# undistro/trivy

Measured on AMD Instinct MI355X. Metric: GB/s secret-scanned (whole node) at 1/2/4/8 MI355X; findings bit-exact vs CPU, higher is better.
Workload: dtype u8

## Files before the change

trivy_amd/csrc/engine.hip:

```cpp
#include <chrono>
#include <condition_variable>
#include <mutex>
#include <hip/hip_runtime.h>

#include <algorithm>
#include <cstdlib>
#include <cstdio>
#include <cstring>
#include <string>
#include <pthread.h>

#include <thread>
#include <type_traits>

#include "engine.h"
#include "census.h"
#include "fetch.h"
#include "fetch_host.h"
#include "fetch_windows.h"
#include "xform.h"
#include "filter.h"
#include "k1_orform.h"

namespace tsg {

namespace {

constexpr int kScanThreads = 1024;
constexpr int kScanWaves = kScanThreads / 64;

#define HIP_OK(x)                                                   \
  do {                                                              \
    hipError_t e_ = (x);                                            \
    if (e_ != hipSuccess) {                                         \
      err_ = std::string(#x) + ": " + hipGetErrorString(e_);        \
      return false;                                                 \
    }                                                               \
  } while (0)


constexpr uint32_t kK0Run = 16;
struct ClearParams {
  uint32_t* flags;
  uint32_t* kw;
  uint64_t n_kw;
  uint32_t* counters;
  uint32_t* fs_ctr;
  uint32_t* skip_info;
};
__device__ __forceinline__ void clear_words(uint32_t* p, uint64_t n, uint64_t tid, uint64_t nthr) {
  const uint64_t n4 = n / 4;
  for (uint64_t i = tid; i < n4; i += nthr) reinterpret_cast<uint4*>(p)[i] = make_uint4(0, 0, 0, 0);
  if (tid < n % 4) p[4 * n4 + tid] = 0;
}
__global__ __launch_bounds__(256) void chunk_map_kernel(const uint64_t* __restrict__ off, uint32_t n_files,
                                                        uint64_t n_chunks, uint32_t* __restrict__ chunk_file,
                                                        ClearParams Z) {
  {
    const uint64_t tid = uint64_t(blockIdx.x) * blockDim.x + threadIdx.x, nthr = uint64_t(gridDim.x) * blockDim.x;
    clear_words(Z.flags, n_files, tid, nthr);
    clear_words(Z.kw, Z.n_kw, tid, nthr);
    if (tid < kScanCtrWords) {
      Z.counters[tid] = 0;
      if (Z.fs_ctr) Z.fs_ctr[tid] = 0;
      if (Z.skip_info) Z.skip_info[tid] = 0;
    }
  }
  const uint64_t n_runs = (n_chunks + kK0Run - 1) / kK0Run;
  for (uint64_t r = uint64_t(blockIdx.x) * blockDim.x + threadIdx.x; r < n_runs;
       r += uint64_t(gridDim.x) * blockDim.x) {
    const uint64_t c0 = r * kK0Run;
    uint64_t x = c0 * kChunk;
    uint32_t lo = 0, hi = n_files;
    while (hi - lo > 1) {
      const uint32_t mid = (lo + hi) >> 1;
      if (off[mid] <= x) lo = mid;
      else hi = mid;
    }
    uint32_t v[kK0Run];
    uint64_t fe = off[lo + 1];
#pragma unroll
    for (uint32_t i = 0; i < kK0Run; i++) {
      x = (c0 + i) * kChunk;
      while (x >= fe && lo + 1 < n_files) fe = off[++lo + 1];
      v[i] = lo;
    }
    if (c0 + kK0Run <= n_chunks) {
      uint4* d = reinterpret_cast<uint4*>(chunk_file + c0);
#pragma unroll
      for (uint32_t q = 0; q < kK0Run / 4; q++) d[q] = make_uint4(v[4 * q], v[4 * q + 1], v[4 * q + 2], v[4 * q + 3]);
    } else {
      for (uint32_t i = 0; c0 + i < n_chunks; i++) chunk_file[c0 + i] = v[i];
    }
  }
}

__device__ __forceinline__ uint4 load16(const uint8_t* p) { return *reinterpret_cast<const uint4*>(p); }

__device__ __forceinline__ void wave_sync() {
  __builtin_amdgcn_fence(__ATOMIC_RELEASE, "wavefront");
  __builtin_amdgcn_wave_barrier();
  __builtin_amdgcn_fence(__ATOMIC_ACQUIRE, "wavefront");
}

constexpr int kFLane = 64;
constexpr int kFBlocks = kFLane / 16;
constexpr int kFTile = 64 * kFLane;
constexpr int kFFlushAt = 128;
constexpr int kFQueue = kFFlushAt + 64;
constexpr int kFChunks = kFTile / 1024;
#ifndef TSG_K1_NLTILES
#define TSG_K1_NLTILES 16
#endif
constexpr int kFNlTiles = TSG_K1_NLTILES;
#ifndef TSG_K1_WGS
#define TSG_K1_WGS 2
#endif
constexpr int kFWgPerCu = TSG_K1_WGS;
constexpr uint32_t kFGroup = 8;
#ifndef TSG_K1_OR_READAHEAD
#define TSG_K1_OR_READAHEAD 4
#endif
constexpr uint32_t kFReadAheadOr = TSG_K1_OR_READAHEAD;
constexpr int kFWindow = 6;
constexpr int kFWords = 4;
static_assert(kChunk % kFLane == 0 && kChunk / kFLane <= 64, "a newline chunk must be whole lane chunks");
static_assert(kFChunks * kChunk == kFTile && kFChunks == 4, "a tile's newline counts are one u64");


constexpr uint32_t kRunWords = 8;
__host__ __device__ inline uint64_t KeepWords(uint64_t n_tiles) {
  return ((n_tiles + 63) / 64 + kRunWords - 1) / kRunWords * kRunWords;
}

__global__ __launch_bounds__(256) void tile_keep_kernel(const uint64_t* __restrict__ off, uint32_t n_files,
                                                        const uint32_t* __restrict__ chunk_file,
                                                        const uint8_t* __restrict__ skip, uint64_t n_bytes,
                                                        uint64_t n_tiles, uint64_t* __restrict__ keep_bits,
                                                        uint32_t* __restrict__ info) {
  const uint32_t lane = threadIdx.x & 63u;
  const uint64_t stride = uint64_t(gridDim.x) * blockDim.x;
  const uint64_t n_padded = KeepWords(n_tiles) * 64;
  for (uint64_t base = uint64_t(blockIdx.x) * blockDim.x + (threadIdx.x & ~63u); base < n_padded; base += stride) {
    const uint64_t t = base + lane;
    bool keep = false;
    if (t < n_tiles) {
      const uint64_t ts = t * kFTile, te = ts + kFTile < n_bytes ? ts + kFTile : n_bytes;
      uint32_t f = chunk_file[t * kFChunks];
      for (;;) {
        const uint64_t fb = off[f], fe = off[f + 1];
        if (fe > fb && !skip[f]) {
          keep = true;
          break;
        }
        if (fe >= te || f + 1 >= n_files) break;
        f++;
      }
    }
    const uint64_t m = __ballot(keep);
    if (lane == 0) keep_bits[base / 64] = m;
  }
  constexpr uint32_t kStatBlocks = 64;
  if (blockIdx.x >= kStatBlocks) return;
  const uint64_t fstride = uint64_t(gridDim.x < kStatBlocks ? gridDim.x : kStatBlocks) * blockDim.x;
  uint32_t nf = 0;
  uint64_t nb = 0;
  for (uint64_t f = uint64_t(blockIdx.x) * blockDim.x + threadIdx.x; f < n_files; f += fstride)
    if (skip[f]) {
      nf++;
      nb += off[f + 1] - off[f];
    }
#pragma unroll
  for (int x = 1; x < 64; x <<= 1) {
    nf += __shfl_xor(nf, x);
    nb += __shfl_xor(nb, x);
  }
  if (lane == 0 && nf) {
    atomicAdd(&info[kSkFiles], nf);
    atomicAdd(reinterpret_cast<unsigned long long*>(&info[kSkBytes]), static_cast<unsigned long long>(nb));
  }
}

constexpr int kRunThreads = 1024;
__global__ __launch_bounds__(kRunThreads) void tile_runs_kernel(const uint64_t* __restrict__ keep_bits,
                                                                uint64_t n_tiles, uint2* __restrict__ runs,
                                                                uint32_t* __restrict__ info) {
  __shared__ uint32_t s_k[kRunThreads / 64], s_r[kRunThreads / 64];
  const uint32_t tid = threadIdx.x, lane = tid & 63u, wv = tid >> 6;
  const uint64_t n_words = KeepWords(n_tiles);
  const uint64_t per = ((n_words / kRunWords + kRunThreads - 1) / kRunThreads) * kRunWords;
  const uint64_t w0 = per * tid < n_words ? per * tid : n_words;
  const uint64_t w1 = w0 + per < n_words ? w0 + per : n_words;
  const uint64_t carry0 = w0 > 0 && w0 < n_words ? keep_bits[w0 - 1] >> 63 : 0;
  auto load_group = [&](uint64_t w, uint64_t* b) {
    const uint4* g = reinterpret_cast<const uint4*>(keep_bits + w);
#pragma unroll
    for (uint32_t q = 0; q < kRunWords / 2; q++) {
      const uint4 v = g[q];
      b[2 * q] = uint64_t(v.x) | (uint64_t(v.y) << 32);
      b[2 * q + 1] = uint64_t(v.z) | (uint64_t(v.w) << 32);
    }
  };
  uint32_t kept = 0, starts = 0;
  uint64_t carry = carry0;
  for (uint64_t w = w0; w < w1; w += kRunWords) {
    uint64_t g[kRunWords];
    load_group(w, g);
#pragma unroll
    for (uint32_t q = 0; q < kRunWords; q++) {
      const uint64_t b = g[q];
      kept += uint32_t(__popcll(b));
      starts += uint32_t(__popcll(b & ~((b << 1) | carry)));
      carry = b >> 63;
    }
  }
  uint32_t ik = kept, ir = starts;
#pragma unroll
  for (int x = 1; x < 64; x <<= 1) {
    const uint32_t a = __shfl_up(ik, x), b = __shfl_up(ir, x);
    if (lane >= uint32_t(x)) {
      ik += a;
      ir += b;
    }
  }
  if (lane == 63) {
    s_k[wv] = ik;
    s_r[wv] = ir;
  }
  __syncthreads();
  uint32_t bk = 0, br = 0;
  for (uint32_t q = 0; q < wv; q++) {
    bk += s_k[q];
    br += s_r[q];
  }
  uint32_t k = bk + ik - kept, r = br + ir - starts;
  carry = carry0;
  for (uint64_t w = w0; w < w1; w += kRunWords) {
    uint64_t g[kRunWords];
    load_group(w, g);
#pragma unroll
    for (uint32_t q = 0; q < kRunWords; q++) {
      const uint64_t b = g[q];
      for (uint64_t s = b & ~((b << 1) | carry); s; s &= s - 1) {
        const uint32_t bit = uint32_t(__builtin_ctzll(s));
        runs[r++] = make_uint2(uint32_t((w + q) * 64 + bit), k + uint32_t(__popcll(b & ((uint64_t(1) << bit) - 1))));
      }
      k += uint32_t(__popcll(b));
      carry = b >> 63;
    }
  }
  if (tid == kRunThreads - 1) {
    runs[r] = make_uint2(uint32_t(n_tiles), k);
    info[kSkRuns] = r;
    info[kSkKept] = k;
    info[kSkTailKept] = n_tiles ? uint32_t((keep_bits[(n_tiles - 1) / 64] >> ((n_tiles - 1) & 63)) & 1) : 0u;
    info[kSkTiles] = uint32_t(n_tiles);
  }
}

struct FilterParams {
  const uint8_t* arena;
  uint64_t n_bytes;
  const uint2* runs;
  uint32_t* run_info;
  const uint32_t* reach;
  uint32_t diag_mode;
  uint16_t* nl;
  uint32_t* recs;
  uint32_t rec_cap;
  uint32_t* counters;
};

__device__ __forceinline__ uint4 reach_read(const uint8_t* sb, uint32_t w, uint32_t k, uint32_t laneoff) {
  return *reinterpret_cast<const uint4*>(sb + __builtin_amdgcn_perm(w, laneoff, 0x0C0C0000u | ((4u + k) << 8)));
}

__device__ __forceinline__ uint4 reach_read_whole(const uint8_t* sb, uint32_t w, uint32_t k, uint32_t laneoff) {
  uint4 r = reach_read(sb, w, k, laneoff);
  asm volatile("" : "+v"(r.x), "+v"(r.y), "+v"(r.z), "+v"(r.w));
  return r;
}

__device__ __forceinline__ void reach_apply(const uint4& m, uint32_t* st) {
  asm("v_lshl_or_b32 %0, %1, 4, %2" : "=v"(st[0]) : "v"(st[0]), "v"(m.x));
  asm("v_lshl_or_b32 %0, %1, 4, %2" : "=v"(st[1]) : "v"(st[1]), "v"(m.y));
  asm("v_lshl_or_b32 %0, %1, 4, %2" : "=v"(st[2]) : "v"(st[2]), "v"(m.z));
  asm("v_lshl_or_b32 %0, %1, 4, %2" : "=v"(st[3]) : "v"(st[3]), "v"(m.w));
}

__device__ __forceinline__ uint32_t nl_count4(uint32_t w) {
  const uint32_t a = ((w ^ 0x0A0A0A0Au) & 0x7F7F7F7Fu) + 0x7F7F7F7Fu;
  return __popc(~(a | w) & 0x80808080u);
}

__device__ __forceinline__ uint32_t word_of(uint4 v, uint32_t i) {
  return i < 2 ? (i == 0 ? v.x : v.y) : (i == 2 ? v.z : v.w);
}

__device__ __forceinline__ void load_reach_lds(uint8_t* s_reach, const uint32_t* reach, int tid, int nthreads) {
  for (uint32_t i = tid; i < 256; i += nthreads)
    reinterpret_cast<uint4*>(s_reach)[i] = reinterpret_cast<const uint4*>(reach)[i];
}

__device__ __forceinline__ void load_orform_lds(uint8_t* s_reach, const uint32_t* reach, int tid, int nthreads) {
  for (uint32_t i = tid; i < 256 * 4; i += nthreads) {
    const uint32_t b = i >> 2;
    const uint4 r = reinterpret_cast<const uint4*>(reach)[b];
    const uint32_t in[4] = {r.x, r.y, r.z, r.w};
    uint32_t w[4];
    OrFormRow(in, w);
#pragma unroll
    for (uint32_t c = 0; c < 4; c++)
      reinterpret_cast<uint4*>(s_reach)[b * 16 + (i & 3) * 4 + c] = make_uint4(w[0], w[1], w[2], w[3]);
  }
}

__device__ __forceinline__ uint32_t or3_keep(uint32_t a, uint32_t b, uint32_t c) {
  uint32_t h;
  asm("v_or3_b32 %0, %1, %2, %3" : "=v"(h) : "v"(a), "v"(b), "v"(c));
  return h;
}
__device__ __forceinline__ uint32_t and_or_keep(uint32_t acc, uint32_t a, uint32_t b) {
  asm("v_bitop3_b32 %0, %1, %2, %3 bitop3:0xe0" : "=v"(acc) : "v"(acc), "v"(a), "v"(b));
  return acc;
}

template <bool kRuns>
__global__ __launch_bounds__(kScanThreads, 8) void filter_kernel(FilterParams P) {
  __shared__ __attribute__((aligned(16))) uint8_t s_reach[65536];
  __shared__ uint32_t s_queue[kScanWaves * kFQueue];
  __shared__ uint64_t s_nl[kScanWaves * kFNlTiles];
  const int tid = threadIdx.x;
  load_orform_lds(s_reach, P.reach, tid, blockDim.x);
  __syncthreads();
  const uint32_t lane = tid & 63;
  const uint32_t wave = __builtin_amdgcn_readfirstlane(uint32_t(tid) >> 6);
  uint32_t* Q = s_queue + wave * kFQueue;
  uint64_t* NL = s_nl + wave * kFNlTiles;
  auto ln = [&]() {
    uint32_t l = lane;
    asm volatile("" : "+v"(l));
    return l;
  };
  uint32_t nl_slots = 0;
  uint32_t qn = 0;
  const uint64_t n_tiles = (P.n_bytes + kFTile - 1) / kFTile;
  const uint64_t n_waves = uint64_t(gridDim.x) * kScanWaves;
  const uint64_t wid = uint64_t(blockIdx.x) * kScanWaves + wave;
  const uint2* __restrict__ RUNS = kRuns ? P.runs : nullptr;
  auto uni = [](uint32_t v) { return uint32_t(__builtin_amdgcn_readfirstlane(v)); };
  const uint64_t n_kept = RUNS ? uint64_t(uni(P.run_info[kSkKept])) : n_tiles;
  const bool tail_kept = RUNS ? uni(P.run_info[kSkTailKept]) != 0 : true;
  const uint64_t per = n_kept / n_waves, extra = n_kept % n_waves;
  auto uni64 = [&](uint64_t v) { return uint64_t(uni(uint32_t(v))) | uint64_t(uni(uint32_t(v >> 32))) << 32; };
  const uint64_t k_begin = uni64(wid * per + (wid < extra ? wid : extra));
  const uint64_t k_end = uni64(k_begin + per + (wid < extra ? 1 : 0));
  uint32_t run = 0;
  uint64_t run_k1 = n_kept;
  uint64_t t_begin = k_begin;
  uint32_t runs_walked = 1;
  if (RUNS && k_begin < k_end) {
    uint32_t lo = 0, hi = uni(P.run_info[kSkRuns]);
    while (hi - lo > 1) {
      const uint32_t mid = (lo + hi) >> 1;
      if (uni(RUNS[mid].y) <= k_begin) lo = mid;
      else hi = mid;
    }
    run = lo;
    const uint2 r0 = RUNS[lo];
    t_begin = uint64_t(uni(r0.x)) + (k_begin - uni(r0.y));
    run_k1 = uni(RUNS[lo + 1].y);
  }
  uint4 buf[kFBlocks];
  uint32_t pre_x = 0, pre_y = 0;
  auto load_pre = [&](uint64_t tt) {
    const uint2 pv = *reinterpret_cast<const uint2*>(P.arena + tt * kFTile - 8);
    pre_x = __builtin_amdgcn_readfirstlane(pv.x);
    pre_y = __builtin_amdgcn_readfirstlane(pv.y);
  };
  if (k_begin < k_end && t_begin > 0) load_pre(t_begin);
  auto next_tile = [&](uint64_t k1, uint64_t tcur, bool* nr) -> uint64_t {
    if (k1 < run_k1) {
      *nr = false;
      return tcur + 1;
    }
    run++;
    runs_walked++;
    run_k1 = uni(RUNS[run + 1].y);
    *nr = true;
    return uni(RUNS[run].x);
  };
  auto lane_ptr = [&](uint64_t tt) -> const uint8_t* {
    const uint64_t b0 = tt * kFTile + uint64_t(ln()) * kFLane;
    return P.arena + (b0 < P.n_bytes ? b0 : 0);
  };
  auto load_tile = [&](uint4* dst, uint64_t tt) {
    const uint8_t* lp = lane_ptr(tt);
#pragma unroll
    for (int j = 0; j < kFBlocks; j++) dst[j] = load16(lp + 16 * j);
  };
  auto flush = [&]() {
    uint32_t base = 0;
    const uint32_t l = ln();
    if (l == 0) base = atomicAdd(&P.counters[kCtRecs], qn);
    base = __builtin_amdgcn_readfirstlane(base);
    for (uint32_t i = l; i < qn; i += 64) {
      if (base + i < P.rec_cap) P.recs[base + i] = Q[i];
      else P.counters[kCtRecOvf] = 1;
    }
    qn = 0;
  };
  uint32_t fl_acc = 0;
  uint32_t grp_n = 0;
  uint64_t grp_t0 = 0;
  auto compact = [&]() {
    const uint32_t cnt = __popc(fl_acc);
    uint32_t incl = cnt;
    incl += uint32_t(__builtin_amdgcn_update_dpp(0, int(incl), 0x111, 0xF, 0xF, true));
    incl += uint32_t(__builtin_amdgcn_update_dpp(0, int(incl), 0x112, 0xF, 0xF, true));
    incl += uint32_t(__builtin_amdgcn_update_dpp(0, int(incl), 0x114, 0xF, 0xF, true));
    incl += uint32_t(__builtin_amdgcn_update_dpp(0, int(incl), 0x118, 0xF, 0xF, true));
    incl += uint32_t(__builtin_amdgcn_update_dpp(0, int(incl), 0x142, 0xA, 0xF, false));
    incl += uint32_t(__builtin_amdgcn_update_dpp(0, int(incl), 0x143, 0xC, 0xF, false));
    const uint32_t total = __builtin_amdgcn_readlane(incl, 63);
    if (total) {
      if (qn + total > kFQueue) flush();
      const uint32_t l = ln();
      const uint32_t rec0 = __builtin_amdgcn_readfirstlane(uint32_t(grp_t0 * (kFTile / 16))) + l * kFBlocks;
      uint32_t m = fl_acc;
      if (total <= kFQueue) {
        uint32_t at = qn + incl - cnt;
        while (m) {
          const uint32_t b = uint32_t(__builtin_ctz(m));
          m &= m - 1;
          Q[at++] = rec0 + ((b >> 2) << 8) + (b & 3u);
        }
        qn += total;
      } else {
        uint32_t base = 0;
        if (l == 0) base = atomicAdd(&P.counters[kCtRecs], total);
        uint32_t at = __builtin_amdgcn_readfirstlane(base) + incl - cnt;
        while (m) {
          const uint32_t b = uint32_t(__builtin_ctz(m));
          m &= m - 1;
          if (at < P.rec_cap) P.recs[at] = rec0 + ((b >> 2) << 8) + (b & 3u);
          else P.counters[kCtRecOvf] = 1;
          at++;
        }
      }
    }
    fl_acc = 0;
    grp_n = 0;
  };
  auto flush_nl = [&](uint64_t t_last) {
    wave_sync();
    uint32_t l = lane;
    asm volatile("" : "+v"(l));
    if (l < nl_slots) {
      const uint64_t tt = t_last - uint64_t(nl_slots - 1 - l);
      reinterpret_cast<uint64_t*>(P.nl)[tt] = NL[l];
    }
    nl_slots = 0;
  };
  auto tile = [&](uint4* cur, uint64_t tt, auto tail_tag, const uint8_t* nxt = nullptr) {
    constexpr bool kTail = decltype(tail_tag)::value;
    constexpr bool kRefill = !kTail;
    if (kTail) {
      const uint64_t b0 = tt * kFTile + uint64_t(lane) * kFLane;
#pragma unroll
      for (int j = 0; j < kFBlocks; j++) {
        const uint64_t p = b0 + 16 * j;
        uint32_t wd[4] = {cur[j].x, cur[j].y, cur[j].z, cur[j].w};
#pragma unroll
        for (int q = 0; q < 4; q++) {
          const uint64_t wp = p + 4 * q;
          if (wp >= P.n_bytes) wd[q] = 0;
          else if (wp + 4 > P.n_bytes) wd[q] &= (1u << (8 * (P.n_bytes - wp))) - 1u;
        }
        cur[j] = make_uint4(wd[0], wd[1], wd[2], wd[3]);
      }
    }
    const uint32_t p0 = uint32_t(__builtin_amdgcn_update_dpp(int(pre_x), int(cur[kFBlocks - 1].z), 0x138, 0xF, 0xF,
                                                             false));
    const uint32_t p1 = uint32_t(__builtin_amdgcn_update_dpp(int(pre_y), int(cur[kFBlocks - 1].w), 0x138, 0xF, 0xF,
                                                             false));
    pre_x = __builtin_amdgcn_readlane(cur[kFBlocks - 1].z, 63);
    pre_y = __builtin_amdgcn_readlane(cur[kFBlocks - 1].w, 63);
    uint32_t flagged = 0, nl = 0;
    if (P.diag_mode < 2) {
      const uint32_t laneoff = (ln() & 15) * 16;
      constexpr uint32_t kRA = kFReadAheadOr;
      static_assert(kRA % 2 == 0 && 16 % kRA == 0, "positions are combined in pairs");
      uint32_t xh[4], yh[2], hprev;
      {
        auto row = [&](uint32_t w, uint32_t k) { return reach_read_whole(s_reach, w, k, laneoff); };
        const uint4 r5 = row(p0, 3), r4 = row(p1, 0), r3 = row(p1, 1), r2 = row(p1, 2), r1 = row(p1, 3);
        hprev = or3_keep(r5.x, r3.y, r1.z);
        xh[0] = r4.x, xh[1] = r3.x, xh[2] = r2.x, xh[3] = r1.x;
        yh[0] = r2.y, yh[1] = r1.y;
      }
#pragma unroll
      for (int j = 0; j < kFBlocks; j++) {
        const uint32_t wd[4] = {cur[j].x, cur[j].y, cur[j].z, cur[j].w};
        uint32_t acc = ~0u;
#pragma unroll
        for (uint32_t g = 0; g < 16; g += kRA) {
          uint4 m[kRA];
#pragma unroll
          for (uint32_t q = 0; q < kRA; q++) m[q] = reach_read(s_reach, wd[(g + q) >> 2], (g + q) & 3, laneoff);
#pragma unroll
          for (uint32_t q = 0; q < kRA; q += 2) {
            const uint32_t k = g + q;
            const uint32_t h0 = or3_keep(xh[k & 3], yh[0], m[q].z);
            const uint32_t h1 = or3_keep(xh[(k + 1) & 3], yh[1], m[q + 1].z);
            xh[k & 3] = m[q].x, xh[(k + 1) & 3] = m[q + 1].x;
            yh[0] = m[q].y, yh[1] = m[q + 1].y;
            const uint32_t hi = __builtin_amdgcn_perm(h1, h0, 0x07060302u);
            const uint32_t lo = __builtin_amdgcn_perm(h0, hprev, 0x05040100u);
            acc = and_or_keep(acc, hi, lo);
            nl += m[q].w + m[q + 1].w;
            hprev = h1;
          }
        }
        flagged |= uint32_t(acc != ~0u) << j;
        if constexpr (kRefill) cur[j] = load16(nxt + 16 * j);
      }
    } else {
#pragma unroll
      for (int j = 0; j < kFBlocks; j++) {
        nl += nl_count4(cur[j].x) + nl_count4(cur[j].y) + nl_count4(cur[j].z) + nl_count4(cur[j].w);
        if constexpr (kRefill) cur[j] = load16(nxt + 16 * j);
      }
    }
    {
    nl += uint32_t(__builtin_amdgcn_update_dpp(0, int(nl), 0x111, 0xF, 0xF, true));
    nl += uint32_t(__builtin_amdgcn_update_dpp(0, int(nl), 0x112, 0xF, 0xF, true));
    nl += uint32_t(__builtin_amdgcn_update_dpp(0, int(nl), 0x114, 0xF, 0xF, true));
    nl += uint32_t(__builtin_amdgcn_update_dpp(0, int(nl), 0x118, 0xF, 0xF, true));
    static_assert(kChunk / kFLane == 16, "one newline chunk per DPP row");
    static_assert(kFTile / 16 == 256, "a tile's records: 256 blocks");
    const uint32_t l = ln();
    if ((l & 15) == 15) reinterpret_cast<uint16_t*>(NL + nl_slots)[l >> 4] = uint16_t(nl);
    if (++nl_slots == kFNlTiles) flush_nl(tt);
    }
    if (grp_n == 0) grp_t0 = tt;
    fl_acc |= flagged << (4 * grp_n);
    grp_n++;
  };
  auto flush_due = [&]() {
    if (grp_n == kFGroup) compact();
    if (qn >= kFFlushAt) flush();
  };
  using Full = std::false_type;
  if constexpr (!kRuns) {
    const uint64_t t_end = k_end;
    const uint64_t t_full = t_end < P.n_bytes / kFTile ? t_end : P.n_bytes / kFTile;
    uint64_t t = t_begin;
    if (t < t_full) load_tile(buf, t);
    while (t < t_full) {
      flush_due();
      tile(buf, t, Full(), lane_ptr(t + 1 < t_full ? t + 1 : t));
      t++;
    }
    if (t < t_end) {
      flush_due();
      load_tile(buf, t);
      tile(buf, t, std::true_type());
      t++;
    }
    if (grp_n) compact();
    if (qn) flush();
    if (nl_slots) flush_nl(t - 1);
    return;
  }
  const bool partial = (P.n_bytes % kFTile) != 0 && tail_kept;
  const uint64_t k_full = uni64((partial && k_end == n_kept && k_end > k_begin) ? k_end - 1 : k_end);
  uint64_t k = k_begin, t = t_begin, t_prev = t_begin;
  bool nr_cur = false;
  auto run_boundary = [&]() {
    if (grp_n) compact();
    if (nl_slots) flush_nl(t_prev);
  };
  auto step = [&](uint4* cur) {
    if (nr_cur) run_boundary();
    flush_due();
    uint64_t tn = t;
    bool nr_n = false;
    if (k + 1 < k_end) tn = next_tile(k + 1, t, &nr_n);
    if (nr_cur) load_pre(t);
    tile(cur, t, Full(), lane_ptr(k + 1 < k_full ? tn : t));
    t_prev = t;
    t = tn;
    nr_cur = nr_n;
    k++;
  };
  if (k < k_full) load_tile(buf, t);
  while (k < k_full) step(buf);
  if (k < k_end) {
    if (nr_cur) run_boundary();
    flush_due();
    if (nr_cur) load_pre(t);
    load_tile(buf, t);
    tile(buf, t, std::true_type());
    t_prev = t;
    k++;
  }
  if (grp_n) compact();
  if (qn) flush();
  if (nl_slots) flush_nl(t_prev);
  if (RUNS && lane == 0 && k_begin < k_end) atomicMax(&P.run_info[kSkWaveRuns], runs_walked);
}

struct NfaParams {
  const uint8_t* arena;
  const uint64_t* off;
  uint32_t n_files;
  const uint16_t* nl;
  const AnchorInfo* anchors;
  const RuleGpu* rules;
  const uint32_t* rule_kw;
  const uint32_t* kwbits;
  uint32_t kw_words;
  const uint32_t* flags;
  const uint64_t* nfa;
  const uint32_t* hits;
  uint32_t hit_cap;
  uint32_t* counters;
  Candidate* cands;
  uint32_t cand_cap;
  const uint32_t* fullscan_rules;
  uint32_t n_fullscan_rules;
  uint32_t fs_chunk;
  uint32_t kw_fold;
  uint32_t diag;
  const uint8_t* skip;
  uint32_t drop_marked;
};

__device__ __forceinline__ bool kw_bits_inexact(const NfaParams& P, uint32_t f) {
  return (P.flags[f] & 4u) && !(P.kw_fold && P.counters[kCtFoldOvf] == 0);
}



#ifndef TSG_C_THREADS
#define TSG_C_THREADS 512
#endif
constexpr int kCThreads = TSG_C_THREADS;
#ifndef TSG_C_THREADS_G
#define TSG_C_THREADS_G 256
#endif
constexpr int kCThreadsG = TSG_C_THREADS_G;
template <bool kLdsTabs>
constexpr int ConfirmThreads() { return kLdsTabs ? kCThreads : kCThreadsG; }

struct FoldSite {
  uint64_t x;
  uint32_t f;
  uint32_t len;
};

__device__ __forceinline__ uint32_t wave_slot(uint32_t* ctr) {
  const uint64_t m = __ballot(1);
  const uint32_t leader = uint32_t(__ffsll(static_cast<unsigned long long>(m)) - 1);
  const uint32_t rank = __builtin_amdgcn_mbcnt_hi(uint32_t(m >> 32), __builtin_amdgcn_mbcnt_lo(uint32_t(m), 0u));
  uint32_t base = 0;
  if (rank == 0) base = atomicAdd(ctr, uint32_t(__popcll(m)));
  base = __shfl(base, int(leader));
  return base + rank;
}

#ifndef TSG_C_HITS
#define TSG_C_HITS 96
#endif
constexpr uint32_t kCWaveHits = TSG_C_HITS;

constexpr uint32_t kHitAidBits = 24;
__device__ __forceinline__ uint32_t hit_aid_word(uint32_t aid, uint64_t end) {
  return aid | (uint32_t(end >> 32) << kHitAidBits);
}
__host__ __device__ __forceinline__ void hit_unpack(const uint32_t* h, uint32_t* f, uint64_t* end, uint32_t* aid) {
  *f = h[0];
  *end = uint64_t(h[1]) | (uint64_t(h[2] >> kHitAidBits) << 32);
  *aid = h[2] & ((1u << kHitAidBits) - 1u);
}

__device__ __forceinline__ void stage_hit(uint32_t* hbuf, uint32_t* hcnt, uint32_t* hits, uint32_t cap,
                                          uint32_t* counters, uint32_t f, uint64_t end, uint32_t aid) {
  const uint32_t k = atomicAdd(hcnt, 1u);
  if (k < kCWaveHits) {
    hbuf[3 * k + 0] = f;
    hbuf[3 * k + 1] = uint32_t(end);
    hbuf[3 * k + 2] = hit_aid_word(aid, end);
    return;
  }
  const uint32_t g = atomicAdd(&counters[kCtHits], 1u);
  if (g < cap) {
    hits[3ull * g + 0] = f;
    hits[3ull * g + 1] = uint32_t(end);
    hits[3ull * g + 2] = hit_aid_word(aid, end);
  } else {
    counters[kCtHitOvf] = 1;
  }
}

__device__ __forceinline__ void flush_staged(uint32_t* hbuf, uint32_t* hcnt, uint32_t* hits, uint32_t cap,
                                             uint32_t* counters, uint32_t lane) {
  wave_sync();
  const uint32_t n_all = __builtin_amdgcn_readfirstlane(*hcnt);
  const uint32_t n = n_all < kCWaveHits ? n_all : kCWaveHits;
  if (n) {
    uint32_t base = 0;
    if (lane == 0) base = atomicAdd(&counters[kCtHits], n);
    base = __builtin_amdgcn_readfirstlane(base);
    for (uint32_t i = lane; i < n; i += 64) {
      if (base + i < cap) {
        hits[3ull * (base + i) + 0] = hbuf[3 * i + 0];
        hits[3ull * (base + i) + 1] = hbuf[3 * i + 1];
        hits[3ull * (base + i) + 2] = hbuf[3 * i + 2];
      } else {
        counters[kCtHitOvf] = 1;
      }
    }
  }
  wave_sync();
  if (lane == 0) *hcnt = 0;
  wave_sync();
}

__device__ __forceinline__ void put_hit(uint32_t* hits, uint32_t cap, uint32_t* counters, uint32_t f, uint64_t end,
                                        uint32_t aid) {
  const uint32_t g = wave_slot(&counters[kCtHits]);
  if (g < cap) {
    hits[3ull * g + 0] = f;
    hits[3ull * g + 1] = uint32_t(end);
    hits[3ull * g + 2] = hit_aid_word(aid, end);
  } else {
    counters[kCtHitOvf] = 1;
  }
}
__device__ __forceinline__ bool follow_lut_pass(const FollowLut& L, const uint32_t* X, int64_t avail) {
  const uint32_t n0 = L.n[0], n1 = L.n[1];
  if (n0 == 0) return true;
  const int64_t span0 = int64_t(L.hi[0]) + n0, span1 = n1 ? int64_t(L.hi[1]) + n1 : 0;
  const int64_t lim = avail < (span0 > span1 ? span0 : span1) ? avail : (span0 > span1 ? span0 : span1);
  uint32_t nonascii = 0;
#pragma unroll
  for (int j = 0; j < 13; j++) {
    const int64_t v = lim - 4 * j;
    const uint32_t vm = v >= 4 ? ~0u : (v <= 0 ? 0u : (1u << (8 * uint32_t(v))) - 1u);
    nonascii |= X[j] & vm;
  }
  if (nonascii & 0x80808080u) return true;
  uint32_t t[4], h[2];
// ... 2682 lines not shown
    fo.n_items = e.n_fitems_;
    fo.stage_items = e.fold_stage_ ? 1u : 0u;
    fo.n_classes = e.n_fclasses_;
    static const uint32_t fold_diag =
        std::getenv("TSG_DIAG_FOLD") ? uint32_t(std::atoi(std::getenv("TSG_DIAG_FOLD"))) : 0u;
    fo.diag = fold_diag;
    fo.pairs = static_cast<const FoldPair*>(e.d_fold_pairs_);
    fo.first = static_cast<const uint32_t*>(e.d_fold_first_);
    fo.n_pairs_k = e.n_fold_pairs_k_;
    fo.n_pairs_s = e.n_fold_pairs_s_;
    fo.n_cap_k = e.n_fold_cap_k_;
    fo.n_cap_s = e.n_fold_cap_s_;
    fo.folds = static_cast<const FoldSite*>(e.d_folds_);
    fo.fold_cap = e.caps_.fold;
    fo.idx_off = static_cast<const uint32_t*>(e.d_fold_idx_off_);
    fo.idx_items = static_cast<const uint32_t*>(e.d_fold_idx_items_);
    fo.n_cap_k_idx = e.n_fold_cap_k_idx_;
    fo.n_cap_s_idx = e.n_fold_cap_s_idx_;
    fo.hits = static_cast<uint32_t*>(e.d_hits_);
    fo.hit_cap = e.caps_.hit;
    fo.counters = W.counters;
    return fo;
  }
  static KwFoldParams KwFold(const GpuEngine& e, const WorkSet& W, const uint8_t* d_arena,
                             const uint64_t* d_offsets) {
    KwFoldParams kf;
    kf.arena = d_arena;
    kf.off = d_offsets;
    kf.tabs = static_cast<const uint8_t*>(e.d_ftabs_);
    kf.t_items = e.ft_items_;
    kf.t_item_ids = e.ft_item_ids_;
    kf.t_item_cls = e.ft_item_cls_;
    kf.t_classes = e.ft_classes_;
    kf.pairs = static_cast<const FoldPair*>(e.d_kwfold_pairs_);
    kf.n_rng_i = e.n_kwf_ri_;
    kf.n_rng_k = e.n_kwf_rk_;
    kf.n_cap_i = e.n_kwf_ci_;
    kf.n_cap_k = e.n_kwf_ck_;
    kf.folds = static_cast<const FoldSite*>(e.d_folds_);
    kf.fold_cap = e.caps_.fold;
    kf.counters = W.counters;
    kf.kwbits = static_cast<uint32_t*>(W.kw);
    kf.kw_words = e.kw_words_;
    return kf;
  }
  static NfaParams Nfa(const GpuEngine& e, const WorkSet& W, const uint8_t* d_arena, const uint64_t* d_offsets,
                       uint32_t n_files, const SkipIn* skip) {
    NfaParams np;
    np.arena = d_arena;
    np.off = d_offsets;
    np.n_files = n_files;
    np.nl = static_cast<const uint16_t*>(e.d_nl_);
    np.anchors = e.d_anchors_;
    np.rules = e.d_rules_;
    np.rule_kw = e.d_rule_kw_;
    np.kwbits = static_cast<const uint32_t*>(W.kw);
    np.kw_words = e.kw_words_;
    np.flags = static_cast<const uint32_t*>(W.flags);
    np.nfa = e.d_nfa_;
    np.hits = static_cast<const uint32_t*>(e.d_hits_);
    np.hit_cap = e.caps_.hit;
    np.counters = W.counters;
    static const uint32_t verify_diag =
        std::getenv("TSG_DIAG_VERIFY") ? uint32_t(std::atoi(std::getenv("TSG_DIAG_VERIFY"))) : 0u;
    np.diag = verify_diag;
    np.cands = static_cast<Candidate*>(W.cands);
    np.cand_cap = e.caps_.cand;
    np.fullscan_rules = e.d_fullscan_rules_;
    np.n_fullscan_rules = e.n_fullscan_rules_;
    np.fs_chunk = e.fs_chunk_;
    np.skip = skip ? skip->d_skip : nullptr;
    np.drop_marked = skip && skip->drop_marked ? 1u : 0u;
    np.kw_fold = e.kw_fold_ ? 1u : 0u;
    return np;
  }
  static FsLists FullScanLists(const GpuEngine& e, const WorkSet& W) {
    FsLists fq;
    fq.pairs = static_cast<FsPair*>(e.d_fs_pairs_);
    fq.pair_cap = e.caps_.fs_pair;
    fq.tasks = static_cast<FsTask*>(e.d_fs_tasks_);
    fq.task_cap = e.caps_.fs_task;
    fq.wave_pairs = static_cast<uint32_t*>(e.d_fs_wave_);
    fq.ctr = W.fs_ctr;
    fq.task_min = e.caps_.fs_task_bytes;
    return fq;
  }
};

bool GpuEngine::EnqueuePhase(const uint8_t* d_arena, uint64_t n_bytes, const uint64_t* d_offsets, uint32_t n_files,
                             uint64_t n_chunks, WorkSet& W, bool k0_aux, PhaseEvents& E, const SkipIn* skip) {
  const uint64_t f_tiles = (n_bytes + kFTile - 1) / kFTile;
  if (skip && (!skip->d_skip || f_tiles == 0)) skip = nullptr;
  if (!EnsureSets(n_chunks, n_files, f_tiles, skip != nullptr)) return false;
  if (!Ensure(&d_nl_, &cap_nl_, (n_chunks + 8) * 2) ||
      !Ensure(&d_folds_, &cap_folds_, size_t(caps_.fold) * sizeof(FoldSite)) ||
      !Ensure(&d_recs_, &cap_recs_, size_t(caps_.rec) * 4) ||
      !Ensure(&d_hits_, &cap_hits_, size_t(caps_.hit) * 12))
    return false;
  if (n_fullscan_rules_ > 0 &&
      (!Ensure(&d_fs_pairs_, &cap_fs_pairs_, size_t(caps_.fs_pair) * sizeof(FsPair)) ||
       !Ensure(&d_fs_wave_, &cap_fs_wave_, size_t(caps_.fs_pair) * 4) ||
       !Ensure(&d_fs_tasks_, &cap_fs_tasks_, size_t(caps_.fs_task) * 4 * sizeof(FsTask))))
    return false;
  const hipStream_t k0s = k0_aux ? aux_stream_ : stream_;
  if (skip && skip->ready) HIP_OK(hipStreamWaitEvent(k0s, skip->ready, 0));
  if (W.free_rec) HIP_OK(hipStreamWaitEvent(k0s, W.free_ev, 0));
  if (!k0_aux && W.k0_rec) HIP_OK(hipStreamWaitEvent(stream_, W.k0_done, 0));
  if (k0_aux && k2_rec_) HIP_OK(hipStreamWaitEvent(aux_stream_, k2_done_, 0));
  if (!k0_aux) {
    HIP_OK(hipEventRecord(E.ev[kEvStart], stream_));
    if (d_item_diag_) HIP_OK(hipMemsetAsync(d_item_diag_, 0, 8 * std::max<size_t>(n_fitems_, 1), stream_));
  }
  HIP_OK(hipEventRecord(E.ev_k0[0], k0s));
  {
    const uint64_t used = (n_bytes + kChunk - 1) / kChunk;
    const uint64_t runs = (used + kK0Run - 1) / kK0Run;
    const uint64_t clear_q = (uint64_t(n_files) * (1 + kw_words_) + 3) / 4;
    const uint64_t work = std::max(runs, clear_q);
    const uint32_t blocks = uint32_t(std::max<uint64_t>(1, std::min<uint64_t>((work + 255) / 256, 8192)));
    ClearParams z;
    z.flags = static_cast<uint32_t*>(W.flags);
    z.kw = static_cast<uint32_t*>(W.kw);
    z.n_kw = uint64_t(n_files) * kw_words_;
    z.counters = W.counters;
    z.fs_ctr = n_fullscan_rules_ > 0 ? W.fs_ctr : nullptr;
    z.skip_info = skip ? W.skip_info : nullptr;
    chunk_map_kernel<<<blocks, 256, 0, k0s>>>(d_offsets, n_files, used, static_cast<uint32_t*>(W.chunk_file), z);
    HIP_OK(hipGetLastError());
  }
  if (skip) {
    const uint32_t blocks =
        uint32_t(std::max<uint64_t>(1, std::min<uint64_t>((KeepWords(f_tiles) * 64 + 255) / 256, 4096)));
    tile_keep_kernel<<<blocks, 256, 0, k0s>>>(d_offsets, n_files, static_cast<const uint32_t*>(W.chunk_file),
                                              skip->d_skip, n_bytes, f_tiles, static_cast<uint64_t*>(W.keep_bits),
                                              W.skip_info);
    HIP_OK(hipGetLastError());
    tile_runs_kernel<<<1, kRunThreads, 0, k0s>>>(static_cast<const uint64_t*>(W.keep_bits), f_tiles,
                                                 static_cast<uint2*>(W.runs), W.skip_info);
    HIP_OK(hipGetLastError());
  }
  HIP_OK(hipEventRecord(E.ev_k0[1], k0s));
  if (k0_aux) {
    HIP_OK(hipEventRecord(W.k0_done, aux_stream_));
    W.k0_rec = true;
    HIP_OK(hipEventRecord(E.ev[kEvStart], stream_));
    if (d_item_diag_) HIP_OK(hipMemsetAsync(d_item_diag_, 0, 8 * std::max<size_t>(n_fitems_, 1), stream_));
    HIP_OK(hipStreamWaitEvent(stream_, W.k0_done, 0));
  }
  const FilterParams fp = KernelArgs::Filter(*this, W, d_arena, n_bytes, skip);
  uint32_t f_grid =
      uint32_t(std::max<uint64_t>(1, std::min<uint64_t>((f_tiles + kScanWaves - 1) / kScanWaves, 256 * kFWgPerCu)));
  if (k1_grid_cap_) f_grid = std::min(f_grid, k1_grid_cap_);
  HIP_OK(hipEventRecord(E.ev[kEvK1], stream_));
  if (skip) filter_kernel<true><<<f_grid, kScanThreads, 0, stream_>>>(fp);
  else filter_kernel<false><<<f_grid, kScanThreads, 0, stream_>>>(fp);
  HIP_OK(hipGetLastError());
  HIP_OK(hipEventRecord(E.ev[kEvK2], stream_));
  const ConfirmParams cp = KernelArgs::Confirm(*this, W, d_arena, n_bytes, d_offsets);
  if (diag_mode_ == 0) {
    if (lds_tabs_)
      confirm_kernel<true><<<2048 * 256 / kCThreads, kCThreads, c_lds_bytes_, stream_>>>(cp);
    else
      confirm_kernel<false><<<2048 * 256 / kCThreadsG, kCThreadsG, c_lds_bytes_, stream_>>>(cp);
  }
  HIP_OK(hipGetLastError());
  HIP_OK(hipEventRecord(E.ev[kEvFold], stream_));
  HIP_OK(hipEventRecord(k2_done_, stream_));
  k2_rec_ = true;
  const FoldParams fo = KernelArgs::Fold(*this, W, d_arena, d_offsets);
  if (diag_mode_ == 0) {
    if (lds_tabs_)
      fold_kernel<true><<<fold_grid_, 64 * kFoldWaves, ftabs_fold_bytes_ + 32 * n_fitems_, stream_>>>(fo);
    else if (fold_stage_)
      fold_kernel<false, 16><<<2048, 64 * 16, fold_stage_bytes_, stream_>>>(fo);
    else
      fold_kernel<false><<<2048, 64 * kFoldWaves, 0, stream_>>>(fo);
  }
  HIP_OK(hipGetLastError());
  if (diag_mode_ == 0 && kw_fold_ && n_kwf_ci_ + n_kwf_ck_ > 0) {
    const KwFoldParams kf = KernelArgs::KwFold(*this, W, d_arena, d_offsets);
    kwfold_kernel<<<1024, 64 * kFoldWaves, 0, stream_>>>(kf);
    HIP_OK(hipGetLastError());
  }
  HIP_OK(hipEventRecord(E.ev[kEvVerify], stream_));
  const NfaParams np = KernelArgs::Nfa(*this, W, d_arena, d_offsets, n_files, skip);
  if (diag_mode_ == 0) verify_hits_kernel<<<verify_blocks_, 256, 0, stream_>>>(np);
  HIP_OK(hipGetLastError());
  if (np.n_fullscan_rules > 0) {
    HIP_OK(hipEventRecord(E.ev_fs, stream_));
    const FsLists fq = KernelArgs::FullScanLists(*this, W);
    const uint64_t pairs = uint64_t(n_files) * n_fullscan_rules_;
    const uint32_t pb = uint32_t(std::min<uint64_t>(std::max<uint64_t>((pairs + 255) / 256, 1), 4096));
    fs_pairs_kernel<<<pb, 256, 0, stream_>>>(np, fq);
    HIP_OK(hipGetLastError());
    fs_task_kernel<<<2048, 256, 0, stream_>>>(np, fq);
    HIP_OK(hipGetLastError());
    fs_wave_kernel<<<1024, 256, 0, stream_>>>(np, fq);
    HIP_OK(hipGetLastError());
  }
  HIP_OK(hipEventRecord(E.ev[kEvFinalize], stream_));
  if (diag_mode_ == 0) finalize_kernel<<<finalize_blocks_, 256, 0, stream_>>>(np);
  HIP_OK(hipGetLastError());
  HIP_OK(hipEventRecord(E.ev[kEvEnd], stream_));
  return true;
}


void FetchOut::Release() {
  if (owner && lease) owner->GiveFetchBuf(lease, lease_cap);
  owner = nullptr;
  lease = nullptr;
  lease_cap = 0;
  buf = nullptr;
}

void GpuEngine::SetFetchSizes(uint64_t stage_bytes, uint64_t direct_bytes) {
  fetch_stage_bytes_.store(std::max<uint64_t>(kFetchSeg, stage_bytes / kFetchSeg * kFetchSeg));
  fetch_direct_bytes_.store(std::max<uint64_t>(1, direct_bytes));
  fetchw_stage_bytes_.store(std::max<uint64_t>(kFetchGranule, stage_bytes / kFetchGranule * kFetchGranule));
}

void* GpuEngine::TakeFetchBuf(size_t need, size_t* cap) { return fetch_pool_->Take(need, cap); }
void GpuEngine::GiveFetchBuf(void* p, size_t cap) { fetch_pool_->Give(p, cap); }

bool GpuEngine::EnsureFetchStream() {
  if (fetch_stream_) return true;
  HIP_OK(hipStreamCreateWithFlags(&fetch_stream_, hipStreamNonBlocking));
  HIP_OK(hipEventCreateWithFlags(&ev_packed_, hipEventDisableTiming));
  HIP_OK(hipEventCreateWithFlags(&ev_drained_, hipEventDisableTiming));
  HIP_OK(hipEventCreate(&ev_run_f_[0]));
  HIP_OK(hipEventCreate(&ev_run_f_[1]));
  HIP_OK(hipMalloc(&d_fctr_, sizeof(FetchCounters)));
  HIP_OK(hipHostMalloc(&h_run_fctr_, sizeof(FetchCounters), hipHostMallocDefault));
  return true;
}

void GpuEngine::NoteFetch(uint64_t packed, uint64_t total) {
  const uint64_t rp = fetch_recent_packed_.load(), rt = fetch_recent_total_.load();
  fetch_recent_packed_.store(std::max(packed, rp - rp / 8));
  fetch_recent_total_.store(std::max(total, rt - rt / 8));
}

bool GpuEngine::IssueFetch(const WorkSet& W, const uint8_t* d_arena, const uint64_t* d_offsets, uint32_t n_files,
                           const uint32_t* h_flags, uint64_t direct, uint64_t stage, uint64_t copy_bytes,
                           uint8_t* h_dst, void* h_ctr, hipEvent_t ev0) {
  if (!EnsureFetchStream()) return false;
  const size_t stage_need = size_t(std::max<uint64_t>(std::min(stage, copy_bytes), 16));
  if (d_fstage_ && cap_fstage_ < stage_need) HIP_OK(hipStreamSynchronize(fetch_stream_));
  if (!Ensure(&d_fscratch_, &cap_fscratch_, FetchScratchBytes(n_files)) ||
      !Ensure(&d_fstage_, &cap_fstage_, stage_need))
    return false;
  FetchCounters* ctr = static_cast<FetchCounters*>(d_fctr_);
  HIP_OK(hipEventRecord(ev0, stream_));
  if (h_flags)
    HIP_OK(hipMemcpyAsync(FetchFlags(d_fscratch_, n_files), h_flags, size_t(n_files) * 4, hipMemcpyHostToDevice,
                          stream_));
  HIP_OK(FetchPlan(h_flags ? nullptr : static_cast<const Candidate*>(W.cands), W.counters + kCtCands, caps_.cand,
                   d_offsets, n_files, direct, d_fscratch_, ctr, stream_));
  HIP_OK(hipMemcpyAsync(h_ctr, ctr, sizeof(FetchCounters), hipMemcpyDeviceToHost, stream_));
  uint8_t* st = static_cast<uint8_t*>(d_fstage_);
  for (uint64_t w0 = 0; w0 < copy_bytes; w0 += stage) {
    const uint64_t w1 = std::min(w0 + stage, copy_bytes);
    HIP_OK(hipStreamWaitEvent(stream_, ev_drained_, 0));
    HIP_OK(FetchPack(d_arena, d_offsets, n_files, d_fscratch_, ctr, w0, w1, st, stream_));
    HIP_OK(hipEventRecord(ev_packed_, stream_));
    HIP_OK(hipStreamWaitEvent(fetch_stream_, ev_packed_, 0));
    HIP_OK(hipMemcpyAsync(h_dst + w0, st, size_t(w1 - w0), hipMemcpyDeviceToHost, fetch_stream_));
    HIP_OK(hipEventRecord(ev_drained_, fetch_stream_));
  }
  if (copy_bytes == 0) {
    HIP_OK(hipEventRecord(ev_packed_, stream_));
    HIP_OK(hipStreamWaitEvent(fetch_stream_, ev_packed_, 0));
  }
  return true;
}

bool GpuEngine::FetchNow(const uint8_t* d_arena, const uint64_t* d_offsets, uint32_t n_files,
                         std::vector<uint8_t> want, bool upload_flags, FetchOut* out) {
  if (!out->h_offsets) {
    err_ = "fetch: the batch's host offsets are missing";
    return false;
  }
  const uint64_t stage = fetch_stage_bytes_.load(), direct = fetch_direct_bytes_.load();
  HostFetchPlan P;
  PlanFetchOnHost(std::move(want), out->h_offsets, n_files, direct, out, &P);
  NoteFetch(P.packed, P.total);
  out->files = out->bytes = out->direct_files = 0;
  out->rounds = 0;
  out->ms_fetch = 0;
  if (P.files == 0) return true;
  if (!EnsureFetchStream()) return false;
  size_t cap = 0;
  void* lease = TakeFetchBuf(size_t(P.total) + 64, &cap);
  if (!lease) {
    err_ = "fetch: hipHostMalloc failed for " + std::to_string(P.total) + " bytes";
    return false;
  }
  out->owner = this;
  out->lease = lease;
  out->lease_cap = cap;
  out->buf = static_cast<const uint8_t*>(lease);
  const uint32_t* h_flags = nullptr;
  if (upload_flags) {
    if (!EnsureHost(&h_fflags_, &cap_h_fflags_, size_t(n_files) * 4 + 4)) return false;
    uint32_t* hf = static_cast<uint32_t*>(h_fflags_);
    for (uint32_t f = 0; f < n_files; f++) hf[f] = out->fetched[f];
    h_flags = hf;
  }
// ... 239 lines not shown
```

Measured before the change: 3169.

## Load per-lane 8-byte prefix with tile instead of DPP shift; template out diag path

Each lane now loads the 8 bytes preceding its chunk alongside the tile loads, replacing the DPP row-shift plus readlane carry and the separate load_pre at run boundaries. The run table is read through the constant address space with 32-bit indices, the diag-mode branch becomes a template parameter, and launch bounds are derived from the workgroups-per-CU setting. Scheduling barriers pin load ordering. This removes cross-lane dependencies and per-tile serial carry at the cost of one extra small global load per lane per tile, and it truncates counters to 32 bits.

```diff
diff --git a/trivy_amd/csrc/engine.hip b/trivy_amd/csrc/engine.hip
--- a/trivy_amd/csrc/engine.hip
+++ b/trivy_amd/csrc/engine.hip
@@ -117,6 +117,7 @@
 #define TSG_K1_WGS 2
 #endif
 constexpr int kFWgPerCu = TSG_K1_WGS;
+constexpr int kFWavesPerSimd = kFWgPerCu * kScanThreads / 256;
 constexpr uint32_t kFGroup = 8;
 #ifndef TSG_K1_OR_READAHEAD
 #define TSG_K1_OR_READAHEAD 4
@@ -325,8 +326,8 @@
   return acc;
 }
 
-template <bool kRuns>
-__global__ __launch_bounds__(kScanThreads, 8) void filter_kernel(FilterParams P) {
+template <bool kRuns, bool kDiag>
+__global__ __launch_bounds__(kScanThreads, kFWavesPerSimd) void filter_kernel(FilterParams P) {
   __shared__ __attribute__((aligned(16))) uint8_t s_reach[65536];
   __shared__ uint32_t s_queue[kScanWaves * kFQueue];
   __shared__ uint64_t s_nl[kScanWaves * kFNlTiles];
@@ -347,7 +348,10 @@
   const uint64_t n_tiles = (P.n_bytes + kFTile - 1) / kFTile;
   const uint64_t n_waves = uint64_t(gridDim.x) * kScanWaves;
   const uint64_t wid = uint64_t(blockIdx.x) * kScanWaves + wave;
-  const uint2* __restrict__ RUNS = kRuns ? P.runs : nullptr;
+  using RunTable = const __attribute__((address_space(4))) uint32_t*;
+  const RunTable RUNS = kRuns ? (RunTable)(P.runs) : nullptr;
+  auto run_tile = [&](uint32_t r) { return uint32_t(__builtin_amdgcn_readfirstlane(RUNS[2 * r])); };
+  auto run_kept = [&](uint32_t r) { return uint32_t(__builtin_amdgcn_readfirstlane(RUNS[2 * r + 1])); };
   auto uni = [](uint32_t v) { return uint32_t(__builtin_amdgcn_readfirstlane(v)); };
   const uint64_t n_kept = RUNS ? uint64_t(uni(P.run_info[kSkKept])) : n_tiles;
   const bool tail_kept = RUNS ? uni(P.run_info[kSkTailKept]) != 0 : true;
@@ -356,48 +360,50 @@
   const uint64_t k_begin = uni64(wid * per + (wid < extra ? wid : extra));
   const uint64_t k_end = uni64(k_begin + per + (wid < extra ? 1 : 0));
   uint32_t run = 0;
-  uint64_t run_k1 = n_kept;
+  uint32_t run_k1 = uint32_t(n_kept);
   uint64_t t_begin = k_begin;
   uint32_t runs_walked = 1;
   if (RUNS && k_begin < k_end) {
     uint32_t lo = 0, hi = uni(P.run_info[kSkRuns]);
     while (hi - lo > 1) {
       const uint32_t mid = (lo + hi) >> 1;
-      if (uni(RUNS[mid].y) <= k_begin) lo = mid;
+      if (run_kept(mid) <= k_begin) lo = mid;
       else hi = mid;
     }
     run = lo;
-    const uint2 r0 = RUNS[lo];
-    t_begin = uint64_t(uni(r0.x)) + (k_begin - uni(r0.y));
-    run_k1 = uni(RUNS[lo + 1].y);
+    t_begin = uint64_t(run_tile(lo)) + (k_begin - run_kept(lo));
+    run_k1 = run_kept(lo + 1);
   }
   uint4 buf[kFBlocks];
-  uint32_t pre_x = 0, pre_y = 0;
-  auto load_pre = [&](uint64_t tt) {
-    const uint2 pv = *reinterpret_cast<const uint2*>(P.arena + tt * kFTile - 8);
-    pre_x = __builtin_amdgcn_readfirstlane(pv.x);
-    pre_y = __builtin_amdgcn_readfirstlane(pv.y);
-  };
-  if (k_begin < k_end && t_begin > 0) load_pre(t_begin);
-  auto next_tile = [&](uint64_t k1, uint64_t tcur, bool* nr) -> uint64_t {
+  uint2 pfx = make_uint2(0, 0);
+  auto next_tile = [&](uint32_t k1, uint64_t tcur, bool* nr) -> uint64_t {
     if (k1 < run_k1) {
       *nr = false;
       return tcur + 1;
     }
     run++;
     runs_walked++;
-    run_k1 = uni(RUNS[run + 1].y);
+    run_k1 = run_kept(run + 1);
     *nr = true;
-    return uni(RUNS[run].x);
+    return run_tile(run);
   };
   auto lane_ptr = [&](uint64_t tt) -> const uint8_t* {
     const uint64_t b0 = tt * kFTile + uint64_t(ln()) * kFLane;
     return P.arena + (b0 < P.n_bytes ? b0 : 0);
   };
+  auto pre_ptr = [&](const uint8_t* lp) -> const uint8_t* { return lp == P.arena ? lp : lp - 8; };
   auto load_tile = [&](uint4* dst, uint64_t tt) {
-    const uint8_t* lp = lane_ptr(tt);
-#pragma unroll
-    for (int j = 0; j < kFBlocks; j++) dst[j] = load16(lp + 16 * j);
+    const uint64_t b0 = tt * kFTile + uint64_t(ln()) * kFLane;
+    const bool has_pre = b0 >= 8 && b0 - 8 < P.n_bytes;
+    const uint2 pv = *reinterpret_cast<const uint2*>(P.arena + (has_pre ? b0 - 8 : 0));
+    const uint8_t* lp = P.arena + (b0 < P.n_bytes ? b0 : 0);
+#pragma unroll
+    for (int j = 0; j < kFBlocks; j++) {
+      __builtin_amdgcn_sched_barrier(0);
+      dst[j] = load16(lp + 16 * j);
+    }
+    __builtin_amdgcn_sched_barrier(0);
+    pfx = has_pre ? pv : make_uint2(0, 0);
   };
   auto flush = [&]() {
     uint32_t base = 0;
@@ -479,15 +485,24 @@
         }
         cur[j] = make_uint4(wd[0], wd[1], wd[2], wd[3]);
       }
-    }
-    const uint32_t p0 = uint32_t(__builtin_amdgcn_update_dpp(int(pre_x), int(cur[kFBlocks - 1].z), 0x138, 0xF, 0xF,
-                                                             false));
-    const uint32_t p1 = uint32_t(__builtin_amdgcn_update_dpp(int(pre_y), int(cur[kFBlocks - 1].w), 0x138, 0xF, 0xF,
-                                                             false));
-    pre_x = __builtin_amdgcn_readlane(cur[kFBlocks - 1].z, 63);
-    pre_y = __builtin_amdgcn_readlane(cur[kFBlocks - 1].w, 63);
+      uint32_t pw[2] = {pfx.x, pfx.y};
+#pragma unroll
+      for (int q = 0; q < 2; q++) {
+        const uint64_t wp = b0 - 8 + 4 * q;
+        if (b0 < 8 || wp >= P.n_bytes) pw[q] = 0;
+        else if (wp + 4 > P.n_bytes) pw[q] &= (1u << (8 * (P.n_bytes - wp))) - 1u;
+      }
+      pfx = make_uint2(pw[0], pw[1]);
+    }
+    const uint32_t p0 = pfx.x, p1 = pfx.y;
+    auto refill = [&](int j) {
+      __builtin_amdgcn_sched_barrier(0);
+      if (j == 0) pfx = *reinterpret_cast<const uint2*>(pre_ptr(nxt));
+      cur[j] = load16(nxt + 16 * j);
+      __builtin_amdgcn_sched_barrier(0);
+    };
     uint32_t flagged = 0, nl = 0;
-    if (P.diag_mode < 2) {
+    if constexpr (!kDiag) {
       const uint32_t laneoff = (ln() & 15) * 16;
       constexpr uint32_t kRA = kFReadAheadOr;
       static_assert(kRA % 2 == 0 && 16 % kRA == 0, "positions are combined in pairs");
@@ -523,13 +538,13 @@
           }
         }
         flagged |= uint32_t(acc != ~0u) << j;
-        if constexpr (kRefill) cur[j] = load16(nxt + 16 * j);
+        if constexpr (kRefill) refill(j);
       }
     } else {
 #pragma unroll
       for (int j = 0; j < kFBlocks; j++) {
         nl += nl_count4(cur[j].x) + nl_count4(cur[j].y) + nl_count4(cur[j].z) + nl_count4(cur[j].w);
-        if constexpr (kRefill) cur[j] = load16(nxt + 16 * j);
+        if constexpr (kRefill) refill(j);
       }
     }
     {
@@ -574,8 +589,10 @@
     return;
   }
   const bool partial = (P.n_bytes % kFTile) != 0 && tail_kept;
-  const uint64_t k_full = uni64((partial && k_end == n_kept && k_end > k_begin) ? k_end - 1 : k_end);
-  uint64_t k = k_begin, t = t_begin, t_prev = t_begin;
+  const uint32_t k_last = uint32_t(k_end);
+  const uint32_t k_full = uni((partial && k_end == n_kept && k_end > k_begin) ? k_last - 1 : k_last);
+  uint32_t k = uint32_t(k_begin);
+  uint64_t t = t_begin, t_prev = t_begin;
   bool nr_cur = false;
   auto run_boundary = [&]() {
     if (grp_n) compact();
@@ -586,8 +603,7 @@
     flush_due();
     uint64_t tn = t;
     bool nr_n = false;
-    if (k + 1 < k_end) tn = next_tile(k + 1, t, &nr_n);
-    if (nr_cur) load_pre(t);
+    if (k + 1 < k_last) tn = next_tile(k + 1, t, &nr_n);
     tile(cur, t, Full(), lane_ptr(k + 1 < k_full ? tn : t));
     t_prev = t;
     t = tn;
@@ -596,10 +612,9 @@
   };
   if (k < k_full) load_tile(buf, t);
   while (k < k_full) step(buf);
-  if (k < k_end) {
+  if (k < k_last) {
     if (nr_cur) run_boundary();
     flush_due();
-    if (nr_cur) load_pre(t);
     load_tile(buf, t);
     tile(buf, t, std::true_type());
     t_prev = t;
@@ -3588,8 +3603,9 @@
       uint32_t(std::max<uint64_t>(1, std::min<uint64_t>((f_tiles + kScanWaves - 1) / kScanWaves, 256 * kFWgPerCu)));
   if (k1_grid_cap_) f_grid = std::min(f_grid, k1_grid_cap_);
   HIP_OK(hipEventRecord(E.ev[kEvK1], stream_));
-  if (skip) filter_kernel<true><<<f_grid, kScanThreads, 0, stream_>>>(fp);
-  else filter_kernel<false><<<f_grid, kScanThreads, 0, stream_>>>(fp);
+  const bool diag = fp.diag_mode >= 2;
+  if (skip) (diag ? filter_kernel<true, true> : filter_kernel<true, false>)<<<f_grid, kScanThreads, 0, stream_>>>(fp);
+  else (diag ? filter_kernel<false, true> : filter_kernel<false, false>)<<<f_grid, kScanThreads, 0, stream_>>>(fp);
   HIP_OK(hipGetLastError());
   HIP_OK(hipEventRecord(E.ev[kEvK2], stream_));
   const ConfirmParams cp = KernelArgs::Confirm(*this, W, d_arena, n_bytes, d_offsets);
```

Result: slower. 2790 (-12.0%).
